# metno/mi-fieldcalc

Hardware: AMD Instinct MI355X
Metric: Mcells/s fused vorticity+divergence, 1440x720x137 grid; % HBM roofline (higher is better)
Workload: dtype f32 in/out, f64 combine; 1 GPU; 1440x720x137 float32 fused relvort+divergence (BASELINE.json configs[2]), one 137-level ensemble member per GPU, inputs ALL_DEFINED and resident in HBM; nx=1440, ny=720, nlev=137, members_per_gpu=1, tuning=default, level_stride_floats=1036800

## Files before the change

include/mifc.h:

```cpp
#ifndef MIFC_H
#define MIFC_H

#include <stddef.h>

#ifdef __cplusplus
extern "C" {
#endif

#define MIFC_ABI_VERSION 1

enum { MIFC_ALL_DEFINED = 0, MIFC_NONE_DEFINED = 1, MIFC_SOME_DEFINED = 2 };
enum { MIFC_MEM_HOST = 0, MIFC_MEM_DEVICE = 1 };

typedef struct mifc_ctx mifc_ctx;

int mifc_abi_version(void);
int mifc_device_count(void);
mifc_ctx* mifc_create(int device);
void mifc_destroy(mifc_ctx* ctx);
const char* mifc_last_error(const mifc_ctx* ctx);
int mifc_set_stream(mifc_ctx* ctx, void* hip_stream);
int mifc_use_own_stream(mifc_ctx* ctx);
int mifc_synchronize(mifc_ctx* ctx);
int mifc_not_built(mifc_ctx* ctx, const char* what);
// ... 156 lines not shown
                             const float* airtemp, const float* rh, const float* sst, const float* p, const float* Pw, const float* aice,
                             const float* depth, float vs, float alpha, float zmin, float zmax, float* icing, int* fdefined, float undef,
                             int memkind);
int mifc_vesselIcingMincog(mifc_ctx* ctx, int nx, int ny, const float* sal, const float* wave, const float* x_wind, const float* y_wind,
                           const float* airtemp, const float* rh, const float* sst, const float* p, const float* Pw, const float* aice,
                           const float* depth, float vs, float alpha, float zmin, float zmax, int alt, float* icing, int* fdefined, float undef,
                           int memkind);
enum { MIFC_ICING_MODSTALL = 1, MIFC_ICING_MINCOG = 2 };
int mifc_vesselIcing_levels(mifc_ctx* ctx, int model, int nlev, int nx, int ny, const float* sal, const float* wave, const float* x_wind,
                            const float* y_wind, const float* airtemp, const float* rh, const float* sst, const float* p, const float* Pw,
                            const float* aice, const float* depth, unsigned int shared_mask, float vs, float alpha, float zmin, float zmax, int alt,
                            float* icing, int* fdefined, float undef, int memkind);

int mifc_vortdiv_levels(mifc_ctx* ctx, int nx, int ny, int nlev, const float* u, const float* v, const float* xmapr, const float* ymapr,
                        float* rvort, float* diverg, int* fdefined, float undef, int memkind);
int mifc_vortdiv_levels_enqueue(mifc_ctx* ctx, int nx, int ny, int nlev, const float* u, const float* v, const float* xmapr, const float* ymapr,
                                float* rvort, float* diverg, const int* fdefined_in, float undef, unsigned long long* n_undefined_dev);

size_t mifc_batch_level_stride(int nx, int ny);
int mifc_vortdiv_levels_strided_enqueue(mifc_ctx* ctx, int nx, int ny, int nlev, const float* u, const float* v, const float* xmapr,
                                        const float* ymapr, float* rvort, float* diverg, size_t in_level_stride, size_t out_level_stride,
                                        const int* fdefined_in, float undef, unsigned long long* n_undefined_dev);

int mifc_vortdiv_ff_levels_enqueue(mifc_ctx* ctx, int nx, int ny, int nlev, const float* u, const float* v, const float* xmapr,
                                   const float* ymapr, float* rvort, float* diverg, float* ff, const int* fdefined_in, float undef,
                                   unsigned long long* n_undefined_dev, unsigned long long* n_undefined_ff_dev);

enum {
  MIFC_OP_RELVORT = 0, MIFC_OP_ABSVORT = 1, MIFC_OP_DIVERGENCE = 2, MIFC_OP_VORTDIV = 3,
  MIFC_OP_GRADIENT_X = 4, MIFC_OP_GRADIENT_Y = 5, MIFC_OP_GRADIENT_ABS = 6, MIFC_OP_GRADIENT_LAPLACE = 7,
  MIFC_OP_GWIND_X = 8, MIFC_OP_GWIND_Y = 9, MIFC_OP_GVORT = 10, MIFC_OP_IGWIND = 11,
  MIFC_OP_JACOBIAN = 13,
  MIFC_OP_ADVECTION = 12, MIFC_OP_TFP = 14, MIFC_OP_QVECTOR = 15, MIFC_OP_SHAPIRO2 = 17
};
int mifc_stencil_levels(mifc_ctx* ctx, int op, int nx, int ny, int nlev, const float* f0, const float* f1, const float* xmapr, const float* ymapr,
                        const float* fcoriolis, float* out0, float* out1, int* fdefined, float undef, int memkind);

int mifc_stencil_levels_enqueue(mifc_ctx* ctx, int op, int nx, int ny, int nlev, const float* f0, const float* f1, const float* xmapr,
                                const float* ymapr, const float* fcoriolis, float* out0, float* out1, const int* fdefined_in, float undef,
                                unsigned long long* n_undefined_dev);
unsigned long long mifc_stencil_count_domain(int op, int nx, int ny);

const char* mifc_last_stencil_form(void);

int mifc_stencil_levels_ex(mifc_ctx* ctx, int op, int nx, int ny, int nlev, const float* f0, const float* f1, const float* f2, const float* xmapr,
                           const float* ymapr, const float* fcoriolis, const float* level_scalars, float scalar, int compute, float* out0,
// ... 61 lines not shown
```

include/mifc_measure.h:

```cpp
#ifndef MIFC_MEASURE_H
#define MIFC_MEASURE_H

#include "mifc.h"

#ifdef __cplusplus
extern "C" {
#endif

int mifc_timing_begin(mifc_ctx* ctx);
float mifc_timing_end_ms(mifc_ctx* ctx);
int mifc_bench_stream2(mifc_ctx* ctx, int variant, int blocks, float* dst0, float* dst1, const float* src0, const float* src1,
                       size_t n_floats);

int mifc_diag_division(mifc_ctx* ctx, const float* a, const float* b, const float* g, float* shared, float* plain, size_t n);

#ifdef __cplusplus
}
#endif

#endif
```

mi-fieldcalc_amd/_capi.py:

```python
import ctypes
import os

_HERE = os.path.dirname(os.path.abspath(__file__))
LIB_PATH = os.environ.get("MIFC_LIB_PATH") or os.path.join(_HERE, "libmifc.so")

c_float_p = ctypes.POINTER(ctypes.c_float)
c_int_p = ctypes.POINTER(ctypes.c_int)
c_u64_p = ctypes.POINTER(ctypes.c_ulonglong)

_T = {
    "ctx": ctypes.c_void_p,
    "i": ctypes.c_int,
    "f": ctypes.c_float,
    "fl": ctypes.c_float,
    "s": ctypes.c_char_p,
    "p": ctypes.c_void_p,
    "pi": ctypes.c_void_p,
    "pu": ctypes.c_void_p,
    "z": ctypes.c_size_t,
    "u64": ctypes.c_ulonglong,
}

SIGNATURES = {
    "mifc_abi_version": ("i", []),
    "mifc_device_count": ("i", []),
    "mifc_create": ("ctx", ["i"]),
    "mifc_destroy": (None, ["ctx"]),
    "mifc_last_error": ("s", ["ctx"]),
    "mifc_set_stream": ("i", ["ctx", "p"]),
    "mifc_use_own_stream": ("i", ["ctx"]),
    "mifc_synchronize": ("i", ["ctx"]),
    "mifc_reload_env": ("i", ["ctx"]),
    "mifc_not_built": ("i", ["ctx", "s"]),
    "mifc_device_alloc": ("p", ["ctx", "z"]),
    "mifc_device_free": ("i", ["ctx", "p"]),
# ... 69 lines not shown
    "mifc_fieldOPERconstant": ("i", ["ctx", "i", "i", "i", "p", "f", "p", "pi", "f", "i"]),
    "mifc_constantOPERfield": ("i", ["ctx", "i", "i", "i", "f", "p", "p", "pi", "f", "i"]),
    "mifc_sumFields": ("i", ["ctx", "i", "i", "p", "i", "p", "pi", "f", "i"]),
    "mifc_meanValue": ("i", ["ctx", "i", "i", "p", "p", "i", "p", "pi", "f", "i"]),
    "mifc_stddevValue": ("i", ["ctx", "i", "i", "p", "p", "i", "p", "pi", "f", "i"]),
    "mifc_extremeValue": ("i", ["ctx", "i", "i", "i", "p", "i", "p", "pi", "f", "i"]),
    "mifc_probability": ("i", ["ctx", "i", "i", "i", "p", "p", "i", "p", "i", "p", "pi", "f", "i"]),
    "mifc_ensembleQuantiles": ("i", ["ctx", "i", "i", "i", "i", "p", "pi", "i", "p", "i", "p", "pi", "f", "i"]),
    "mifc_neighbourProbFunctions": ("i", ["ctx", "i", "i", "p", "p", "i", "i", "p", "pi", "f", "i"]),
    "mifc_neighbourFunctions": ("i", ["ctx", "i", "i", "p", "p", "i", "i", "p", "pi", "f", "i"]),
    "mifc_neighbour_levels": ("i", ["ctx", "i", "i", "i", "i", "i", "p", "p", "i", "p", "pi", "f", "i"]),
    "mifc_vesselIcingModStall": ("i", ["ctx", "i", "i"] + ["p"] * 11 + ["f", "f", "f", "f", "p", "pi", "f", "i"]),
    "mifc_vesselIcingMincog": ("i", ["ctx", "i", "i"] + ["p"] * 11 + ["f", "f", "f", "f", "i", "p", "pi", "f", "i"]),
    "mifc_vesselIcing_levels": ("i", ["ctx", "i", "i", "i", "i"] + ["p"] * 11 + ["i", "f", "f", "f", "f", "i", "p", "pi", "f", "i"]),
    "mifc_vortdiv_levels": ("i", ["ctx", "i", "i", "i", "p", "p", "p", "p", "p", "p", "pi", "f", "i"]),
    "mifc_stencil_levels": ("i", ["ctx", "i", "i", "i", "i", "p", "p", "p", "p", "p", "p", "p", "pi", "f", "i"]),
    "mifc_vortdiv_ff_levels_enqueue": ("i", ["ctx", "i", "i", "i", "p", "p", "p", "p", "p", "p", "p", "pi", "f", "pu", "pu"]),
    "mifc_stencil_levels_enqueue": ("i", ["ctx", "i", "i", "i", "i", "p", "p", "p", "p", "p", "p", "p", "pi", "f", "pu"]),
    "mifc_stencil_count_domain": ("u64", ["i", "i", "i"]),
    "mifc_last_stencil_form": ("s", []),
    "mifc_stencil_levels_ex": ("i", ["ctx", "i", "i", "i", "i", "p", "p", "p", "p", "p", "p", "p", "f", "i", "p", "p", "pi", "f", "i"]),
    "mifc_vortdiv_levels_enqueue": ("i", ["ctx", "i", "i", "i", "p", "p", "p", "p", "p", "p", "pi", "f", "pu"]),
    "mifc_batch_level_stride": ("z", ["i", "i"]),
    "mifc_vortdiv_levels_strided_enqueue": ("i", ["ctx", "i", "i", "i", "p", "p", "p", "p", "p", "p", "z", "z", "pi", "f", "pu"]),
    "mifc_hlevel_derived_levels": (
        "i",
        ["ctx", "i", "i", "i", "p", "p", "p", "p", "p", "p", "p", "p", "p", "p", "pi", "pi", "pi", "pi", "pi", "f", "i"],
    ),
    "mifc_hlevel_derived_levels_enqueue": (
        "i",
        ["ctx", "i", "i", "i", "p", "p", "p", "p", "p", "p", "p", "p", "p", "p", "pi", "pi", "f", "pu"],
    ),
    "mifc_hlevel_derived_batch": (
        "i",
        ["ctx", "i", "i", "i", "p", "p", "p", "p", "p", "p", "p", "p", "p", "s", "i", "p", "s", "i", "p", "s", "i", "p", "pi", "pi", "pi", "pi", "pi",
         "pi", "pi", "f", "i"],
    ),
    "mifc_hlevel_derived_batch_enqueue": (
        "i",
        ["ctx", "i", "i", "i", "p", "p", "p", "p", "p", "p", "p", "p", "p", "s", "i", "p", "s", "i", "p", "s", "i", "p", "pi", "pi", "f", "pu"],
    ),
    "mifc_vortdiv_slab_enqueue": ("i", ["ctx", "i", "i", "i", "i", "p", "p", "p", "p", "p", "p", "i", "f", "pu"]),
    "mifc_vortdiv_slab_rows_enqueue": ("i", ["ctx", "i", "i", "i", "i", "i", "i", "p", "p", "p", "p", "p", "p", "i", "f", "pu", "i"]),
    "mifc_halo_copy_enqueue": ("i", ["ctx", "p", "ctx", "p", "z"]),
    "mifc_graph_begin": ("i", ["ctx", "i"]),
    "mifc_graph_begin_lanes": ("i", ["ctx", "i", "i"]),
    "mifc_graph_lane": ("i", ["ctx", "i"]),
    "mifc_graph_end": ("p", ["ctx"]),
    "mifc_graph_launch": ("i", ["p"]),
    "mifc_graph_destroy": (None, ["p"]),
    "mifc_comm_unique_id": ("i", ["p"]),
    "mifc_comm_init": ("i", ["ctx", "p", "i", "i"]),
    "mifc_comm_adopt": ("i", ["ctx", "p"]),
    "mifc_comm_release": ("i", ["ctx"]),
    "mifc_comm_info": ("i", ["ctx", "pi", "pi"]),
    "mifc_slab_plan_create": ("p", ["ctx", "i", "i", "i", "i", "i", "p", "p", "p", "p", "p", "p", "i", "f", "pu"]),
    "mifc_slab_plan_destroy": (None, ["p"]),
    "mifc_slab_plan_step": ("i", ["p"]),
    "mifc_slab_plan_uses_graph": ("i", ["p"]),
    "mifc_slab_plan_begin": ("i", ["p"]),
    "mifc_slab_plan_finish": ("i", ["p"]),
}


MEASURE_SIGNATURES = {
    "mifc_timing_begin": ("i", ["ctx"]),
    "mifc_timing_end_ms": ("fl", ["ctx"]),
    "mifc_bench_stream2": ("i", ["ctx", "i", "i", "p", "p", "p", "p", "z"]),
    "mifc_diag_division": ("i", ["ctx", "p", "p", "p", "p", "p", "z"]),
}


def load_library(path=LIB_PATH):
    if not os.path.exists(path):
        raise ImportError(
            "%s not found: build the HIP extension first (python -c 'import __graft_entry__ as g; g.build()' "
            "or make -C mi-fieldcalc_amd). There is no CPU fallback." % path
        )
    try:
        import torch
    except ImportError:
        pass
    lib = ctypes.CDLL(path)
    for name, (res, args) in SIGNATURES.items():
        fn = getattr(lib, name)
        fn.restype = _T[res] if res else None
        fn.argtypes = [_T[a] for a in args]
    for name, (res, args) in MEASURE_SIGNATURES.items():
        fn = getattr(lib, name, None)
        if fn is not None:
            fn.restype = _T[res] if res else None
            fn.argtypes = [_T[a] for a in args]
# ... 12 lines not shown
```

mi-fieldcalc_amd/csrc/mifc_capi.hip:

```cpp

#include <cmath>
#include <cstdio>
#include <cstdlib>
#include <cstring>
#include <new>
#include <string>
#include <vector>

#include "mifc_ctx.h"

namespace mifc_host {

void stencil_partials(mifc_ctx* c, mifc::StencilParams& P)
{
  P.partials = nullptr;
  P.partials_cap = 0;
  if (P.every_level_all_defined || c->capturing)
    return;
  const size_t per_level = (size_t)(P.ny_local / 4 + 2) * (size_t)(P.nx / 256 + 1);
  const size_t units = per_level * (size_t)P.nlev;
  if (per_level < 2048 || units > ((size_t)1 << 24))
    return;
  int cap = 0;
  P.partials = partials_for(c, units * 1024, &cap);
// ... 1297 lines not shown
  if (timed) {
    (void)hipEventRecord(c->tev[2 * c->n_timed + 1], c->stream);
    c->n_timed += 1;
  }
  if (e != hipSuccess) {
    fail(c, "mifc_vortdiv_ff_levels_enqueue: launch", e);
    return 0;
  }
  if (!every_all && !scratch_release(c))
    return 0;
  return 1;
}

const char* mifc_last_stencil_form(void)
{
  return mifc::last_form();
}

unsigned long long mifc_stencil_count_domain(int op, int nx, int ny)
{
  return stencil_denominator(op, nx, ny);
}

size_t mifc_batch_level_stride(int nx, int ny)
{
  if (nx <= 0 || ny <= 0)
    return 0;
  return mifc::padded_level_stride((size_t)nx * (size_t)ny);
}

static int stencil_enqueue(mifc_ctx* c, const char* who, mifc::StencilParams& P, const int* fdefined_in, unsigned long long* n_undefined_dev)
{
  if (!ensure_levels(c, (size_t)P.nlev))
    return 0;
  bool every_all = (fdefined_in != nullptr), any_all = false;
  for (int l = 0; l < P.nlev; ++l) {
    const bool a = fdefined_in && fdefined_in[l] == MIFC_ALL_DEFINED;
    every_all = every_all && a;
    any_all = any_all || a;
  }
  P.every_level_all_defined = every_all ? 1 : 0;
  P.all_defined = any_all ? c->d_flags : nullptr;
  P.n_undefined = n_undefined_dev;
  if (!every_all && !n_undefined_dev) {
    c->err = std::string(who) + ": n_undefined_dev is required unless every level is ALL_DEFINED";
    return 0;
// ... 511 lines not shown
  if (src_ctx->device == dst_ctx->device)
    MIFC_HIP(dst_ctx, hipMemcpyAsync(dst_dev, src_dev, n_floats * sizeof(float), hipMemcpyDeviceToDevice, dst_ctx->stream));
  else
    MIFC_HIP(dst_ctx, hipMemcpyPeerAsync(dst_dev, dst_ctx->device, src_dev, src_ctx->device, n_floats * sizeof(float), dst_ctx->stream));
  return 1;
}

#ifdef MIFC_MEASUREMENT_BUILD
int mifc_bench_stream2(mifc_ctx* c, int variant, int blocks, float* dst0, float* dst1, const float* src0, const float* src1, size_t n_floats)
{
  CTX_OR_FAIL(c);
  if (n_floats % 4 != 0)
    return 0;
  MIFC_HIP(c, mifc::launch_stream2(variant, blocks, dst0, dst1, src0, src1, n_floats, c->stream));
  return 1;
}

int mifc_diag_division(mifc_ctx* c, const float* a, const float* b, const float* g, float* shared, float* plain, size_t n)
{
  CTX_OR_FAIL(c);
  MIFC_HIP(c, mifc::launch_division_check(a, b, g, shared, plain, n, c->stream));
  return 1;
}
#endif

}
```

mi-fieldcalc_amd/csrc/mifc_kernels.h:

```cpp
#ifndef MIFC_KERNELS_H
#define MIFC_KERNELS_H

#include <hip/hip_runtime.h>

#include "mifc_env.h"

namespace mifc {

typedef unsigned long long u64;

enum EwiseOp {
  EW_VECTORABS = 0,
  EW_TEMP = 1,
  EW_HUM = 2,
  EW_CVHUM_TD = 3,
  EW_CVHUM_RH = 4,
  EW_MOMENTUM_X = 5,
  EW_MOMENTUM_Y = 6,
  EW_TEMP_SCALAR = 7,
  EW_TEMP_PLAIN = 8,
  EW_HUM_DIRECT = 9
};
enum PressureSource { PS_SCALAR = 0, PS_HYBRID = 1, PS_FIELD = 2 };
enum HumKind { HUM_Q_RH = 0, HUM_RH_Q = 1, HUM_Q_TD = 2, HUM_RH_TD = 3 };
// ... 13 lines not shown
  float p;
  float pidcp;
  float pi;
  float tconv;
  float tdconv;
  float alevel, blevel;
  float unit_scale;
  int nx;
  int cell0;
  float fcormin;
  float undef;
  const float* in0;
  const float* in1;
  const float* in2;
  float* out;
  u64* n_undefined;
  unsigned int* partials;
  int partials_cap;
};

hipError_t launch_ewise(const EwiseParams& prm, hipStream_t stream);

size_t padded_level_stride(size_t n);

struct DerivedParams
{
  int n;
  int nlev;
  const float *u, *v, *t, *h, *ps;
  const float *alevel, *blevel;
  float *ff, *temp, *hum, *td;
  float* dd;
  int temp_compute;
  int hum_code, td_code;
  float hum_tdconv, td_tdconv;
  const unsigned char* wind_all_defined;
  const unsigned char* thermo_all_defined;
  int every_level_all_defined;
  float undef;
  u64 *cnt_ff, *cnt_temp, *cnt_hum, *cnt_td, *cnt_dd;
  int n_inline;
  float a_inline[8], b_inline[8];
  unsigned char wind_inline[8], thermo_inline[8];
};
hipError_t launch_derived_levels(const DerivedParams& prm, hipStream_t stream);

// ... 289 lines not shown
```

mi-fieldcalc_amd/csrc/mifc_vortdiv.hip:

```cpp
#include "mifc_device.h"
#include "mifc_kernels.h"

#include <cstdlib>
#include <cstring>
#include <type_traits>

namespace mifc {

namespace {

struct RowsParams
{
  int nx;
  int nyg;
  int j0;
  int ny_local;
  int lo, hi;
  int R;
  int nbands, nwc, nlev;
  int wpb;
  int uL, uB, uW;
  int n_logical;
  int per_xcd;
  int order;
  int xcd_remap;
  int zigzag;
  int nt_interior;
  int lgroup;
#ifdef MIFC_MEASUREMENT_BUILD
  int exp_nohalo;
  int exp_nostore;
  int exp_noload;
  int exp_store_aux;
#endif
  long idx_lo, idx_hi;
  const float *u, *v, *xm, *ym;
  const float* fc;
  float *rv, *dv;
  float* ff;
  u64* n_undefined_ff;
  long in_stride, out_stride;
  const unsigned char* all_defined;
  float undef;
  u64* n_undefined;
  unsigned int* partials;
};

typedef float v4f __attribute__((ext_vector_type(4)));

__device__ __forceinline__ float dpp_from_lower_lane(float keep_if_none, float x)
{
  return __builtin_bit_cast(float,
// ... 845 lines not shown
            if (bottom)
              store4<NT>(dv + oo + nx, d4);
          }
        }
        if (CHECK && P.n_undefined && !all && __builtin_amdgcn_ballot_w64(bad != 0) != 0) {
          const unsigned int n = wave_sum(bad);
          if (lane == 0)
            atomicAdd(&sbad[(lev - lev0) & 1], n);
        }
      }
    }
  }
chunk_done:;
  if (CHECK) {
    asm volatile("s_waitcnt lgkmcnt(0)\n\ts_barrier" ::: "memory");
    if (P.n_undefined && threadIdx.x == 0 && lev1 > lev0) {
      const unsigned int n = sbad[(lev1 - 1 - lev0) & 1];
      if (n != 0)
        atomicAdd(P.n_undefined + (lev1 - 1), (u64)n);
    }
  }
}

template <bool CHECK, bool NT, int TR, int NL, int PF, bool WANT_V = true, bool WANT_D = true, bool ABSV = false, bool FF = false, bool RAGGED = false,
          bool JAC = false>
__global__ __launch_bounds__(64 * (TR + NL)) void vortdiv_split_kernel(const RowsParams P)
{
  static_assert(WANT_V || WANT_D, "nothing to compute");
  static_assert(!JAC || (WANT_V && !WANT_D && !ABSV && !FF), "the Jacobian is a single-output operator");
  static_assert(!(RAGGED && FF), "the three-output form takes aligned fields only");
  static_assert(!FF || (WANT_V && WANT_D && !ABSV), "the wind speed rides on the fused pair");
  static_assert(!ABSV || (WANT_V && !WANT_D), "absvort is a single-output operator");
  constexpr int NB = PF + 1;
  constexpr int NS = TR + 2;
  constexpr int KMAX = (NS + NL - 1) / NL;
  static_assert(4 * NS <= 64, "the edge scalars of a level are one dword per lane");
  static_assert(NL >= 2, "loader 0 gathers the edge scalars, the last loader hands the undefined counts over");
  __shared__ v4f srow[NB][NS][2][64];
  __shared__ float sedge[NB][64];
  __shared__ unsigned int sbad[2];
  __shared__ unsigned int sbadf[2];
  if (CHECK && threadIdx.x < 2) {
    sbad[threadIdx.x] = 0;
    sbadf[threadIdx.x] = 0;
  }
  const int wave = __builtin_amdgcn_readfirstlane((int)(threadIdx.x >> 6));
  const int lane = threadIdx.x & 63;
  const int bid = blockIdx.x;
  const int seq = P.xcd_remap ? ((bid & 7) * P.per_xcd + (bid >> 3)) : bid;
  if (seq >= P.n_logical)
    return;
  const int ntiles = P.uB * P.uW;
  const int lchunk = seq / ntiles;
  const int tile = seq - lchunk * ntiles;
  const int rblock = tile / P.uW;
  const int wc = tile - rblock * P.uW;
  const int lev0 = lchunk * P.lgroup;
  const int lev1 = (lev0 + P.lgroup < P.nlev) ? lev0 + P.lgroup : P.nlev;
  const int nx = P.nx;
  const int first = P.lo + rblock * TR;
  const int col = wc * 256 + lane * 4;
  const bool act = col < nx;
  const int col_c = act ? col : (RAGGED ? 0 : nx - 4);
  const int nvalid = RAGGED ? ((nx - col) < 4 ? (nx - col) : 4) : 4;
  int east_col = wc * 256 + 256;
  if (east_col > nx)
    east_col = nx;

  if (wave >= TR) {
    const int lw = wave - TR;
    int off[KMAX], slot_of[KMAX];
    int off_end[KMAX];
    bool fix[KMAX];
#pragma unroll
    for (int k = 0; k < KMAX; ++k) {
      int s = lw + NL * k;
      if (s > NS - 1)
        s = NS - 1;
      const int jl_raw = first + s - 1;
      const int jl = jl_raw < P.hi ? jl_raw : P.hi;
      slot_of[k] = s;
      off[k] = jl * nx + col_c;
      fix[k] = RAGGED && ((long)off[k] + 3 > P.idx_hi);
      off_end[k] = fix[k] ? (int)P.idx_hi - 3 : off[k];
    }
    const int ei = (lane < 4 * NS) ? lane : 0;
    const int es = ei >> 2;
    const bool e_is_v = ((ei >> 1) & 1) != 0;
    const int ejl_raw = first + es - 1;
    const int ejl = ejl_raw < P.hi ? ejl_raw : P.hi;
    long e64 = (long)ejl * nx + ((ei & 1) ? east_col : (wc * 256 - 1));
    e64 = e64 < P.idx_lo ? P.idx_lo : (e64 > P.idx_hi ? P.idx_hi : e64);
    const int eoff = (int)e64;
    const float* __restrict__ ebase = e_is_v ? P.v : P.u;

    auto walk = [&](auto edge_tag) __attribute__((always_inline)) {
      constexpr bool EDGE = decltype(edge_tag)::value;
      constexpr int L = 2 * KMAX + (EDGE ? 1 : 0);
      auto issue = [&](int lev, int b) {
        const int l = lev < lev1 ? lev : lev1 - 1;
        const float* __restrict__ u = P.u + (size_t)l * P.in_stride;
        const float* __restrict__ v = P.v + (size_t)l * P.in_stride;
        const bool at_end = RAGGED && l == P.nlev - 1;
#pragma unroll
        for (int k = 0; k < KMAX; ++k) {
          const int o = at_end ? off_end[k] : off[k];
          __builtin_amdgcn_global_load_lds((const void __attribute__((address_space(1)))*)(u + o),
                                           (void __attribute__((address_space(3)))*)&srow[b][slot_of[k]][0][0], 16, 0, 0);
          __builtin_amdgcn_global_load_lds((const void __attribute__((address_space(1)))*)(v + o),
                                           (void __attribute__((address_space(3)))*)&srow[b][slot_of[k]][1][0], 16, 0, 0);
        }
        if (EDGE)
          __builtin_amdgcn_global_load_lds((const void __attribute__((address_space(1)))*)(ebase + (size_t)l * P.in_stride + eoff),
                                           (void __attribute__((address_space(3)))*)&sedge[b][0], 4, 0, 0);
        if constexpr (RAGGED) {
          bool mine = false;
#pragma unroll
          for (int k = 0; k < KMAX; ++k)
            mine = mine | fix[k];
          if (at_end && __builtin_amdgcn_ballot_w64(mine) != 0) {
            asm volatile("s_waitcnt vmcnt(0)" ::: "memory");
#pragma unroll
            for (int k = 0; k < KMAX; ++k) {
              if (fix[k]) {
                v4f qu = {0.f, 0.f, 0.f, 0.f}, qv = qu;
#pragma unroll
                for (int c = 0; c < 4; ++c) {
                  const long i = (long)off[k] + c;
                  if (i <= P.idx_hi) {
                    qu[c] = u[i];
                    qv[c] = v[i];
                  }
                }
                srow[b][slot_of[k]][0][lane] = qu;
                srow[b][slot_of[k]][1][lane] = qv;
              }
            }
          }
        }
      };
#pragma unroll
      for (int k = 0; k < PF; ++k)
        issue(lev0 + k, k);
      int b_next = PF % NB;
      auto hand_over = [&](int lev_done) {
        if (CHECK && !EDGE && lw == NL - 1 && P.n_undefined && lane == 0) {
          const int q = (lev_done - lev0) & 1;
          const unsigned int n = sbad[q];
          if (P.partials) {
            P.partials[(size_t)lev_done * (size_t)ntiles + tile] = n;
            if (n != 0)
              sbad[q] = 0;
          } else if (n != 0) {
            atomicAdd(P.n_undefined + lev_done, (u64)n);
            sbad[q] = 0;
          }
          if constexpr (FF) {
            const unsigned int nf = sbadf[q];
            if (nf != 0) {
              atomicAdd(P.n_undefined_ff + lev_done, (u64)nf);
              sbadf[q] = 0;
            }
          }
        }
      };
      for (int lev = lev0; lev < lev1; ++lev) {
        asm volatile("s_waitcnt vmcnt(%0) lgkmcnt(0)\n\ts_barrier" ::"n"((PF - 1) * L) : "memory");
        issue(lev + PF, b_next);
        b_next = (b_next + 1 == NB) ? 0 : b_next + 1;
        if (lev > lev0)
          hand_over(lev - 1);
      }
      asm volatile("s_waitcnt vmcnt(0)" ::: "memory");
      if (CHECK) {
        asm volatile("s_barrier" ::: "memory");
        if (lev1 > lev0)
          hand_over(lev1 - 1);
      }
    };
    if (lw == 0)
      walk(std::true_type());
    else
      walk(std::false_type());
    return;
  }

  const int slot = wave + 1;
  const int jl_raw = first + wave;
  const bool computes = jl_raw < P.hi;
  const int jl = computes ? jl_raw : P.hi;
  const int j = P.j0 + jl;
  const float undef = P.undef;
  const int base = jl * nx;
  const int o = base + col_c;
  const bool top = (j == 1) && (P.j0 == 0);
  const bool bottom = (j == P.nyg - 2) && (P.j0 + P.ny_local == P.nyg);
  const bool last_in_seg = col + 4 >= east_col;
  const int oo = base + col;
  v4f xm4 = {0.f, 0.f, 0.f, 0.f}, ym4 = xm4, fc4 = xm4;
  if (computes) {
    if constexpr (RAGGED) {
      xm4 = reinterpret_cast<const V4Unaligned*>(P.xm + o)->v;
      ym4 = reinterpret_cast<const V4Unaligned*>(P.ym + o)->v;
      if constexpr (ABSV)
        fc4 = reinterpret_cast<const V4Unaligned*>(P.fc + o)->v;
    } else {
      xm4 = load4(P.xm + o);
      ym4 = load4(P.ym + o);
      if constexpr (ABSV)
        fc4 = load4(P.fc + o);
    }
  }
  const int k_last = nx - 1 - col;
  auto fill_columns = [&](float (&z)[4]) __attribute__((always_inline)) {
    if (col == 0)
      z[0] = z[1];
    if constexpr (RAGGED) {
      const float below = dpp_from_lower_lane(z[3], z[3]);
      if (k_last == 0)
        z[0] = below;
      else if (k_last == 1)
        z[1] = z[0];
      else if (k_last == 2)
// ... 26 lines not shown
          store4<NT>(field + oo + nx, z4);
      }
    }
  };
  float hx4[4] = {0.f, 0.f, 0.f, 0.f}, hy4[4] = {0.f, 0.f, 0.f, 0.f};
  bool halves = false;
  if constexpr (JAC) {
    bool exact = true;
#pragma unroll
    for (int k = 0; k < 4; ++k) {
      hx4[k] = 0.5f * xm4[k];
      hy4[k] = 0.5f * ym4[k];
      exact = exact & (__builtin_fabsf(xm4[k]) >= 0x1p-125f || xm4[k] == 0.f) & (__builtin_fabsf(ym4[k]) >= 0x1p-125f || ym4[k] == 0.f);
    }
    halves = __builtin_amdgcn_ballot_w64(!exact) == 0;
  }
  int buf = 0;
  for (int lev = lev0; lev < lev1; ++lev) {
    bool all = true;
    if (CHECK)
      all = level_flag_then_barrier(P.all_defined, lev);
    else
      asm volatile("s_waitcnt lgkmcnt(0)\n\ts_barrier" ::: "memory");
    if (computes) {
      const v4f uc = srow[buf][slot][0][lane], vc = srow[buf][slot][1][lane];
      const float uWe = sedge[buf][4 * slot + 0], uEe = sedge[buf][4 * slot + 1];
      const float vWe = sedge[buf][4 * slot + 2], vEe = sedge[buf][4 * slot + 3];
      const float uW = dpp_from_lower_lane(uWe, uc.w), vW = dpp_from_lower_lane(vWe, vc.w);
      float uE = dpp_from_upper_lane(uEe, uc.x), vE = dpp_from_upper_lane(vEe, vc.x);
      if (last_in_seg) {
        uE = uEe;
        vE = vEe;
      }
      bool ok[4] = {true, true, true, true};
      unsigned int bad = 0;
      if constexpr (JAC) {
        const v4f un = srow[buf][slot + 1][0][lane], us = srow[buf][slot - 1][0][lane];
        const v4f vn = srow[buf][slot + 1][1][lane], vs = srow[buf][slot - 1][1][lane];
        const float ucx[6] = {uW, uc.x, uc.y, uc.z, uc.w, uE};
        const float vcx[6] = {vW, vc.x, vc.y, vc.z, vc.w, vE};
        bool dux[6] = {true, true, true, true, true, true}, dvx[6] = {true, true, true, true, true, true};
        if (CHECK) {
#pragma unroll
          for (int k = 0; k < 6; ++k) {
            dux[k] = __builtin_islessgreater(ucx[k], undef);
            dvx[k] = __builtin_islessgreater(vcx[k], undef);
// ... 87 lines not shown
            f4.x = f[0];
            f4.y = f[1];
            f4.z = f[2];
            f4.w = f[3];
            store4<NT>(ffp + at, f4);
          }
        };
        speed_row(uc, vc, oo);
        if (top)
          speed_row(srow[buf][slot - 1][0][lane], srow[buf][slot - 1][1][lane], oo - nx);
        if (bottom)
          speed_row(srow[buf][slot + 1][0][lane], srow[buf][slot + 1][1][lane], oo + nx);
        if (CHECK && P.n_undefined_ff && !all && __builtin_amdgcn_ballot_w64(badf != 0) != 0) {
          const unsigned int n = wave_sum(badf);
          if (lane == 0)
            atomicAdd(&sbadf[(lev - lev0) & 1], n);
        }
      }
    }
    buf = (buf + 1 == NB) ? 0 : buf + 1;
  }
  if (CHECK)
    asm volatile("s_waitcnt lgkmcnt(0)\n\ts_barrier" ::: "memory");
}

struct Tuning
{
  int K;
  int R;
  int D;
  int NT;
  int V;
  int ORDER;
  int XCD;
  int WPB;
  int ZZ;
  int NTI;
  int XH;
  int XS;
  int PADROWS;
  int XL;
  int LDSX;
  int STA;
  int LG;
  int RB;
};

int tune_value(const char* s, const char* key, int dflt)
{
  const size_t n = std::strlen(key);
  for (const char* p = s; p && *p;) {
    if (std::strncmp(p, key, n) == 0 && p[n] == '=')
      return std::atoi(p + n + 1);
    p = std::strchr(p, ',');
    if (p)
      ++p;
  }
  return dflt;
}

Tuning current_tuning(int nx)
{
  Tuning t = {0, 8, 1, 1, 2, 1, 1, 8, 1, 0, 0, 0, 0, 0, 0, 0, 0, 8};
  if (env().has_vortdiv_tune) {
    const char* s = env().vortdiv_tune;
    t.K = tune_value(s, "K", t.K);
    t.R = tune_value(s, "R", t.R);
    t.D = tune_value(s, "D", t.D);
    t.NT = tune_value(s, "NT", t.NT);
    t.V = tune_value(s, "V", t.V);
    t.ORDER = tune_value(s, "ORDER", t.ORDER);
    t.XCD = tune_value(s, "XCD", t.XCD);
    t.WPB = tune_value(s, "WPB", t.WPB);
    t.ZZ = tune_value(s, "ZZ", t.ZZ);
    t.NTI = tune_value(s, "NTI", t.NTI);
    t.LDSX = tune_value(s, "LDSX", t.LDSX);
    t.LG = tune_value(s, "LG", t.LG);
    t.RB = tune_value(s, "RB", t.RB);
#ifdef MIFC_MEASUREMENT_BUILD
    t.XH = tune_value(s, "XH", 0);
    t.XS = tune_value(s, "XS", 0);
    t.PADROWS = tune_value(s, "PADROWS", 0);
    t.XL = tune_value(s, "XL", 0);
    t.STA = tune_value(s, "STA", 0);
#endif
  }
  if (t.WPB != 1 && t.WPB != 2 && t.WPB != 4 && t.WPB != 8)
    t.WPB = 4;
  if (t.V != 1 && t.V != 2 && t.V != 3)
    t.V = 2;
  if (nx <= 256)
    t.V = 1;
  if (t.R < 1)
    t.R = 1;
  const int rmax = 32 / t.V;
  if (t.R > rmax)
    t.R = rmax;
  if (t.D < 0)
    t.D = 0;
  if (t.D > 1)
    t.D = 1;
  return t;
}

template <bool CHECK, bool WV, bool WD, bool ABSV, int D, bool NT>
void launch_v(const RowsParams& rp, const Tuning& t, int grid, hipStream_t stream)
{
// ... 34 lines not shown
}

template <bool CHECK>
void launch_outputs(const RowsParams& rp, const Tuning& t, int grid, hipStream_t stream)
{
  if (rp.fc)
    launch_d<CHECK, true, false, true>(rp, t, grid, stream);
  else if (rp.rv && rp.dv)
    launch_d<CHECK, true, true, false>(rp, t, grid, stream);
  else if (rp.rv)
    launch_d<CHECK, true, false, false>(rp, t, grid, stream);
  else
    launch_d<CHECK, false, true, false>(rp, t, grid, stream);
}

constexpr int kLevelWalkMinLevels = 3;
constexpr long kLevelWalkMinUnits = 768;

inline bool aligned16(const void* p)
{
  return (reinterpret_cast<size_t>(p) & 15u) == 0;
}

}

size_t padded_level_stride(size_t n)
{
  const size_t n4 = (n + 3) & ~size_t(3);
  return n4;
}

hipError_t launch_vortdiv_rows(const StencilParams& prm, hipStream_t stream, bool* handled)
{
  *handled = false;
  float* rv = nullptr;
  float* dv = nullptr;
  if (prm.op == ST_VORTDIV) {
    rv = prm.out0;
    dv = prm.out1;
  } else if (prm.op == ST_RELVORT) {
    rv = prm.out0;
  } else if (prm.op == ST_DIVERGENCE) {
    dv = prm.out0;
  } else if (prm.op == ST_ABSVORT) {
    rv = prm.out0;
    if (!prm.fcoriolis)
// ... 67 lines not shown
  }
  const bool has_north_halo = prm.j0 > 0;
  const bool has_south_halo = prm.j0 + rp.ny_local < rp.nyg;
  rp.idx_lo = has_north_halo ? -(long)nx : 0;
  rp.idx_hi = (long)nx * (rp.ny_local + (has_south_halo ? 1 : 0)) - 1;
  rp.R = t.R;
  rp.nbands = (rp.hi - rp.lo + t.R - 1) / t.R;
  rp.nwc = (nx + 256 * t.V - 1) / (256 * t.V);
  rp.nlev = prm.nlev;
  rp.wpb = t.WPB;
  rp.uL = (prm.nlev + t.WPB - 1) / t.WPB;
  rp.uB = rp.nbands;
  rp.uW = rp.nwc;
  const long n_logical = (long)rp.uL * rp.uB * rp.uW;
  if (n_logical > 0x3fffffffL)
    return hipSuccess;
  rp.n_logical = (int)n_logical;
  rp.per_xcd = (rp.n_logical + 7) / 8;
  rp.order = t.ORDER;
  rp.xcd_remap = t.XCD;
  rp.zigzag = t.ZZ;
  rp.nt_interior = t.NTI;
  rp.lgroup = t.LG > 0 ? t.LG : 0;
#ifdef MIFC_MEASUREMENT_BUILD
  rp.exp_nohalo = t.XH;
  rp.exp_nostore = t.XS;
  rp.exp_noload = t.XL;
  rp.exp_store_aux = t.STA;
#endif
  rp.u = prm.f0;
  rp.v = prm.f1;
  rp.xm = prm.xmapr;
  rp.ym = prm.ymapr;
  rp.fc = (prm.op == ST_ABSVORT) ? prm.fcoriolis : nullptr;
  rp.rv = rv;
  rp.dv = dv;
  rp.ff = prm.out_ff;
  rp.n_undefined_ff = prm.n_undefined_ff;
  rp.in_stride = prm.in_level_stride;
  rp.out_stride = prm.out_level_stride;
  rp.all_defined = prm.all_defined;
  rp.undef = prm.undef;
  rp.n_undefined = prm.n_undefined;
  rp.partials = nullptr;
  auto counts_by_partials = [&](long units_per_level, bool level_walking = false) {
    const bool yes = prm.partials && prm.n_undefined && !prm.every_level_all_defined && !prm.out_ff && (level_walking || rp.lgroup == 0) &&
                     units_per_level >= 2048 && units_per_level * prm.nlev <= prm.partials_cap;
// ... 154 lines not shown
      } else if (NWsel == 12 && pf == 2) {
        LEVELWALK(12, 2);
      } else if (NWsel == 12) {
        LEVELWALK(12, 1);
      } else if (pf == 2) {
        LEVELWALK(8, 2);
      } else {
        LEVELWALK(8, 1);
      }
#undef LEVELWALK
      return hipGetLastError();
    }
    *handled = false;
    return hipSuccess;
  }
  if (t.K == 4 && prm.op == ST_JACOBIAN && env().has_vortdiv_tune) {
    *handled = false;
    return hipSuccess;
  }
  if (t.K == 4) {
    const bool single = !(rv && dv) || rp.fc;
    const int tile_rows = (single || ragged || prm.out_ff) ? 12 : ((t.RB == 6 || t.RB == 8 || t.RB == 12 || t.RB == 14) ? t.RB : 10);
    const int nchunks_lg = (t.LG > 0 && t.LG < prm.nlev) ? t.LG : prm.nlev;
    const int nchunks = (prm.nlev + nchunks_lg - 1) / nchunks_lg;
    const long units = (long)nchunks * ((rp.hi - rp.lo + tile_rows - 1) / tile_rows) * ((nx + 255) / 256);
    if (units > 0x3fffffffL || (long)nx * (rp.ny_local + 2) >= 0x7fffffffL) {
      *handled = false;
      return hipSuccess;
    }
    rp.uB = (rp.hi - rp.lo + tile_rows - 1) / tile_rows;
    rp.uW = (nx + 255) / 256;
    rp.lgroup = nchunks_lg;
    rp.n_logical = (int)units;
    rp.per_xcd = (rp.n_logical + 7) / 8;
    grid = rp.per_xcd * 8;
    const bool chk = !prm.every_level_all_defined;
    const bool partials = counts_by_partials((long)rp.uB * rp.uW, true);
    auto finish = [&]() {
      if (partials)
        (void)launch_count_partials_levels(prm.partials, rp.uB * rp.uW, prm.nlev, prm.n_undefined, stream);
      return hipGetLastError();
    };
    const int pf = t.D >= 2 ? 3 : (t.D == 1 ? 2 : 1);
    const int nl = (t.WPB == 2 || t.WPB == 4) ? t.WPB : (tile_rows == 10 ? 4 : 2);
#define SPLIT_AS(TR_, NL_, PF_, ...)                                                                                                       \
  if (chk)                                                                                                                                 \
    hipLaunchKernelGGL((vortdiv_split_kernel<true, true, TR_, NL_, PF_, ##__VA_ARGS__>), dim3(grid), dim3(64 * (TR_ + NL_)), 0, stream, rp); \
  else                                                                                                                                     \
    hipLaunchKernelGGL((vortdiv_split_kernel<false, true, TR_, NL_, PF_, ##__VA_ARGS__>), dim3(grid), dim3(64 * (TR_ + NL_)), 0, stream, rp)
    if (prm.out_ff) {
      SPLIT_AS(12, 2, 2, true, true, false, true);
      return finish();
    }
    if (prm.op == ST_JACOBIAN) {
      if (ragged) {
        SPLIT_AS(12, 2, 2, true, false, false, false, true, true);
      } else {
// ... 123 lines not shown
```

Baseline: 374,200 Mcells/s.

## Add balanced level-chunk planning and drain-tail pipeline for split vortdiv kernel

Adds a cost-based planner that picks how many level chunks to split the 137 levels into so work divides evenly across CUs. It also adds a class-based block decoder that spreads long and short chunks and narrow edge columns evenly across XCDs. The loader loop gets a drain tail that no longer issues dead prefetch loads past the chunk end, plus optional masking of loads from inactive lanes. Most of this sits behind tuning keys (BAL, DL, ML) that default to 0. The default path now skips dead prefetches and uses the new tail waits, and it gains measurement-only timing probes.

```diff
diff --git a/include/mifc.h b/include/mifc.h
--- a/include/mifc.h
+++ b/include/mifc.h
@@ -202,6 +202,8 @@
                                         const float* ymapr, float* rvort, float* diverg, size_t in_level_stride, size_t out_level_stride,
                                         const int* fdefined_in, float undef, unsigned long long* n_undefined_dev);
 
+int mifc_plan_level_chunks(long tiles, int nlev, int cus, int* first_level, int cap);
+
 int mifc_vortdiv_ff_levels_enqueue(mifc_ctx* ctx, int nx, int ny, int nlev, const float* u, const float* v, const float* xmapr,
                                    const float* ymapr, float* rvort, float* diverg, float* ff, const int* fdefined_in, float undef,
                                    unsigned long long* n_undefined_dev, unsigned long long* n_undefined_ff_dev);
diff --git a/include/mifc_measure.h b/include/mifc_measure.h
--- a/include/mifc_measure.h
+++ b/include/mifc_measure.h
@@ -14,6 +14,8 @@
 
 int mifc_diag_division(mifc_ctx* ctx, const float* a, const float* b, const float* g, float* shared, float* plain, size_t n);
 
+void mifc_measure_split_probe(unsigned long long* dev);
+
 #ifdef __cplusplus
 }
 #endif
diff --git a/mi-fieldcalc_amd/_capi.py b/mi-fieldcalc_amd/_capi.py
--- a/mi-fieldcalc_amd/_capi.py
+++ b/mi-fieldcalc_amd/_capi.py
@@ -11,6 +11,7 @@
 _T = {
     "ctx": ctypes.c_void_p,
     "i": ctypes.c_int,
+    "l": ctypes.c_long,
     "f": ctypes.c_float,
     "fl": ctypes.c_float,
     "s": ctypes.c_char_p,
@@ -126,6 +127,7 @@
     "mifc_stencil_levels_ex": ("i", ["ctx", "i", "i", "i", "i", "p", "p", "p", "p", "p", "p", "p", "f", "i", "p", "p", "pi", "f", "i"]),
     "mifc_vortdiv_levels_enqueue": ("i", ["ctx", "i", "i", "i", "p", "p", "p", "p", "p", "p", "pi", "f", "pu"]),
     "mifc_batch_level_stride": ("z", ["i", "i"]),
+    "mifc_plan_level_chunks": ("i", ["l", "i", "i", "pi", "i"]),
     "mifc_vortdiv_levels_strided_enqueue": ("i", ["ctx", "i", "i", "i", "p", "p", "p", "p", "p", "p", "z", "z", "pi", "f", "pu"]),
     "mifc_hlevel_derived_levels": (
         "i",
@@ -172,6 +174,7 @@
     "mifc_timing_end_ms": ("fl", ["ctx"]),
     "mifc_bench_stream2": ("i", ["ctx", "i", "i", "p", "p", "p", "p", "z"]),
     "mifc_diag_division": ("i", ["ctx", "p", "p", "p", "p", "p", "z"]),
+    "mifc_measure_split_probe": (None, ["pu"]),
 }
 
 
diff --git a/mi-fieldcalc_amd/csrc/mifc_capi.hip b/mi-fieldcalc_amd/csrc/mifc_capi.hip
--- a/mi-fieldcalc_amd/csrc/mifc_capi.hip
+++ b/mi-fieldcalc_amd/csrc/mifc_capi.hip
@@ -1343,6 +1343,19 @@
   return stencil_denominator(op, nx, ny);
 }
 
+int mifc_plan_level_chunks(long tiles, int nlev, int cus, int* first_level, int cap)
+{
+  if (tiles < 1 || nlev < 1 || cus < 1)
+    return 0;
+  const int n = mifc::plan_level_chunks(tiles, nlev, cus);
+  if (first_level) {
+    const int q = nlev / n, rem = nlev % n;
+    for (int c = 0; c <= n && c < cap; ++c)
+      first_level[c] = c * q + (c < rem ? c : rem);
+  }
+  return n;
+}
+
 size_t mifc_batch_level_stride(int nx, int ny)
 {
   if (nx <= 0 || ny <= 0)
@@ -1900,6 +1913,11 @@
   MIFC_HIP(c, mifc::launch_division_check(a, b, g, shared, plain, n, c->stream));
   return 1;
 }
+
+void mifc_measure_split_probe(unsigned long long* dev)
+{
+  mifc::set_split_probe(dev);
+}
 #endif
 
 }
diff --git a/mi-fieldcalc_amd/csrc/mifc_kernels.h b/mi-fieldcalc_amd/csrc/mifc_kernels.h
--- a/mi-fieldcalc_amd/csrc/mifc_kernels.h
+++ b/mi-fieldcalc_amd/csrc/mifc_kernels.h
@@ -59,6 +59,10 @@
 hipError_t launch_ewise(const EwiseParams& prm, hipStream_t stream);
 
 size_t padded_level_stride(size_t n);
+int plan_level_chunks(long tiles, int nlev, int cus);
+#ifdef MIFC_MEASUREMENT_BUILD
+void set_split_probe(unsigned long long* dev);
+#endif
 
 struct DerivedParams
 {
diff --git a/mi-fieldcalc_amd/csrc/mifc_vortdiv.hip b/mi-fieldcalc_amd/csrc/mifc_vortdiv.hip
--- a/mi-fieldcalc_amd/csrc/mifc_vortdiv.hip
+++ b/mi-fieldcalc_amd/csrc/mifc_vortdiv.hip
@@ -27,7 +27,13 @@
   int zigzag;
   int nt_interior;
   int lgroup;
+  int nchunks;
+  int cls_n[4];
+  int dead_loads;
+  int mask_lanes;
 #ifdef MIFC_MEASUREMENT_BUILD
+  int exp_nodead;
+  unsigned long long* probe;
   int exp_nohalo;
   int exp_nostore;
   int exp_noload;
@@ -919,6 +925,89 @@
   }
 }
 
+struct SplitUnit
+{
+  int lchunk, rblock, wc, lev0, lev1;
+  bool valid;
+};
+__device__ __forceinline__ SplitUnit decode_split_unit(const RowsParams& P, int bid)
+{
+  SplitUnit U;
+  U.valid = false;
+  U.lchunk = U.rblock = U.wc = U.lev0 = U.lev1 = 0;
+  if (P.nchunks > 0) {
+    const int x = bid & 7;
+    int k = bid >> 3, cls = -1;
+#pragma unroll
+    for (int c = 0; c < 4; ++c) {
+      const long n = P.cls_n[c];
+      const int s0 = (int)((x * n) >> 3), s1 = (int)(((x + 1) * n) >> 3);
+      if (cls < 0) {
+        if (k < s1 - s0) {
+          cls = c;
+          k += s0;
+        } else {
+          k -= s1 - s0;
+        }
+      }
+    }
+    if (cls < 0)
+      return U;
+    const bool narrow = cls >= 2, shorter = (cls & 1) != 0;
+    const int has_narrow = (P.cls_n[2] + P.cls_n[3]) > 0 ? 1 : 0;
+    const int wcount = narrow ? 1 : P.uW - has_narrow;
+    const int per_chunk = P.uB * wcount;
+    const int cc = k / per_chunk;
+    const int t = k - cc * per_chunk;
+    U.rblock = t / wcount;
+    U.wc = (narrow ? P.uW - 1 : 0) + (t - U.rblock * wcount);
+    const int q = P.nlev / P.nchunks, rem = P.nlev - q * P.nchunks;
+    U.lchunk = cc + (shorter ? rem : 0);
+    U.lev0 = U.lchunk * q + (U.lchunk < rem ? U.lchunk : rem);
+    U.lev1 = U.lev0 + q + (U.lchunk < rem ? 1 : 0);
+    U.valid = true;
+    return U;
+  }
+  const int seq = P.xcd_remap ? ((bid & 7) * P.per_xcd + (bid >> 3)) : bid;
+  if (seq >= P.n_logical)
+    return U;
+  const int ntiles = P.uB * P.uW;
+  U.lchunk = seq / ntiles;
+  const int tile = seq - U.lchunk * ntiles;
+  U.rblock = tile / P.uW;
+  U.wc = tile - U.rblock * P.uW;
+  U.lev0 = U.lchunk * P.lgroup;
+  U.lev1 = (U.lev0 + P.lgroup < P.nlev) ? U.lev0 + P.lgroup : P.nlev;
+  U.valid = true;
+  return U;
+}
+
+#ifdef MIFC_MEASUREMENT_BUILD
+unsigned long long* g_split_probe = nullptr;
+inline unsigned long long* split_probe_buffer()
+{
+  return g_split_probe;
+}
+constexpr int kSplitProbeWords = 16;
+__device__ __forceinline__ unsigned long long probe_now()
+{
+  return __builtin_amdgcn_s_memtime();
+}
+#define SPLIT_PROBE(word, value)            \
+  do {                                      \
+    if (P.probe && pw >= 0 && lane == 0)    \
+      sprobe[pw][word] = (value);           \
+  } while (0)
+#define SPLIT_PROBE_FLUSH()                                                                  \
+  do {                                                                                       \
+    if (P.probe && pw >= 0 && lane < kSplitProbeWords)                                       \
+      P.probe[((size_t)bid * 3 + pw) * kSplitProbeWords + lane] = sprobe[pw][lane];          \
+  } while (0)
+#else
+#define SPLIT_PROBE(word, value) ((void)0)
+#define SPLIT_PROBE_FLUSH() ((void)0)
+#endif
+
 template <bool CHECK, bool NT, int TR, int NL, int PF, bool WANT_V = true, bool WANT_D = true, bool ABSV = false, bool FF = false, bool RAGGED = false,
           bool JAC = false>
 __global__ __launch_bounds__(64 * (TR + NL)) void vortdiv_split_kernel(const RowsParams P)
@@ -941,23 +1030,30 @@
     sbad[threadIdx.x] = 0;
     sbadf[threadIdx.x] = 0;
   }
+#ifdef MIFC_MEASUREMENT_BUILD
+  const unsigned long long t_start = probe_now();
+#endif
   const int wave = __builtin_amdgcn_readfirstlane((int)(threadIdx.x >> 6));
   const int lane = threadIdx.x & 63;
   const int bid = blockIdx.x;
-  const int seq = P.xcd_remap ? ((bid & 7) * P.per_xcd + (bid >> 3)) : bid;
-  if (seq >= P.n_logical)
+  const SplitUnit U = decode_split_unit(P, bid);
+  if (!U.valid)
     return;
+#ifdef MIFC_MEASUREMENT_BUILD
+  __shared__ unsigned long long sprobe[3][kSplitProbeWords];
+  const int pw = wave == TR ? 0 : (wave == TR + NL - 1 ? 1 : (wave == 0 ? 2 : -1));
+  if (P.probe && pw >= 0 && lane < kSplitProbeWords)
+    sprobe[pw][lane] = 0;
+#endif
   const int ntiles = P.uB * P.uW;
-  const int lchunk = seq / ntiles;
-  const int tile = seq - lchunk * ntiles;
-  const int rblock = tile / P.uW;
-  const int wc = tile - rblock * P.uW;
-  const int lev0 = lchunk * P.lgroup;
-  const int lev1 = (lev0 + P.lgroup < P.nlev) ? lev0 + P.lgroup : P.nlev;
+  const int rblock = U.rblock, wc = U.wc;
+  const int tile = rblock * P.uW + wc;
+  const int lev0 = U.lev0, lev1 = U.lev1;
   const int nx = P.nx;
   const int first = P.lo + rblock * TR;
   const int col = wc * 256 + lane * 4;
   const bool act = col < nx;
+  const bool ld_act = act || !P.mask_lanes;
   const int col_c = act ? col : (RAGGED ? 0 : nx - 4);
   const int nvalid = RAGGED ? ((nx - col) < 4 ? (nx - col) : 4) : 4;
   int east_col = wc * 256 + 256;
@@ -999,13 +1095,15 @@
         const float* __restrict__ u = P.u + (size_t)l * P.in_stride;
         const float* __restrict__ v = P.v + (size_t)l * P.in_stride;
         const bool at_end = RAGGED && l == P.nlev - 1;
-#pragma unroll
-        for (int k = 0; k < KMAX; ++k) {
-          const int o = at_end ? off_end[k] : off[k];
-          __builtin_amdgcn_global_load_lds((const void __attribute__((address_space(1)))*)(u + o),
-                                           (void __attribute__((address_space(3)))*)&srow[b][slot_of[k]][0][0], 16, 0, 0);
-          __builtin_amdgcn_global_load_lds((const void __attribute__((address_space(1)))*)(v + o),
-                                           (void __attribute__((address_space(3)))*)&srow[b][slot_of[k]][1][0], 16, 0, 0);
+        if (ld_act) {
+#pragma unroll
+          for (int k = 0; k < KMAX; ++k) {
+            const int o = at_end ? off_end[k] : off[k];
+            __builtin_amdgcn_global_load_lds((const void __attribute__((address_space(1)))*)(u + o),
+                                             (void __attribute__((address_space(3)))*)&srow[b][slot_of[k]][0][0], 16, 0, 0);
+            __builtin_amdgcn_global_load_lds((const void __attribute__((address_space(1)))*)(v + o),
+                                             (void __attribute__((address_space(3)))*)&srow[b][slot_of[k]][1][0], 16, 0, 0);
+          }
         }
         if (EDGE)
           __builtin_amdgcn_global_load_lds((const void __attribute__((address_space(1)))*)(ebase + (size_t)l * P.in_stride + eoff),
@@ -1036,9 +1134,11 @@
           }
         }
       };
+      const bool dead = P.dead_loads != 0;
 #pragma unroll
       for (int k = 0; k < PF; ++k)
-        issue(lev0 + k, k);
+        if (dead || lev0 + k < lev1)
+          issue(lev0 + k, k);
       int b_next = PF % NB;
       auto hand_over = [&](int lev_done) {
         if (CHECK && !EDGE && lw == NL - 1 && P.n_undefined && lane == 0) {
@@ -1061,12 +1161,39 @@
           }
         }
       };
-      for (int lev = lev0; lev < lev1; ++lev) {
+      int lev = lev0;
+      for (; lev + PF < lev1; ++lev) {
         asm volatile("s_waitcnt vmcnt(%0) lgkmcnt(0)\n\ts_barrier" ::"n"((PF - 1) * L) : "memory");
+        SPLIT_PROBE(lev == lev0 ? 1 : 2, probe_now());
+        if (lev - lev0 < 8)
+          SPLIT_PROBE(8 + lev - lev0, probe_now());
         issue(lev + PF, b_next);
         b_next = (b_next + 1 == NB) ? 0 : b_next + 1;
         if (lev > lev0)
           hand_over(lev - 1);
+      }
+#pragma unroll
+      for (int r = PF - 1; r >= 0; --r) {
+        if (lev1 - lev0 > r) {
+          bool keep_wait = dead;
+#ifdef MIFC_MEASUREMENT_BUILD
+          keep_wait = keep_wait || P.exp_nodead != 0;
+#endif
+          if (keep_wait)
+            asm volatile("s_waitcnt vmcnt(%0) lgkmcnt(0)\n\ts_barrier" ::"n"((PF - 1) * L) : "memory");
+          else
+            asm volatile("s_waitcnt vmcnt(%0) lgkmcnt(0)\n\ts_barrier" ::"n"(r * L) : "memory");
+          SPLIT_PROBE(lev == lev0 ? 1 : 2, probe_now());
+          if (lev - lev0 < 8)
+            SPLIT_PROBE(8 + lev - lev0, probe_now());
+          if (dead) {
+            issue(lev + PF, b_next);
+            b_next = (b_next + 1 == NB) ? 0 : b_next + 1;
+          }
+          if (lev > lev0)
+            hand_over(lev - 1);
+          ++lev;
+        }
       }
       asm volatile("s_waitcnt vmcnt(0)" ::: "memory");
       if (CHECK) {
@@ -1074,7 +1201,21 @@
         if (lev1 > lev0)
           hand_over(lev1 - 1);
       }
+      SPLIT_PROBE(3, probe_now());
+      SPLIT_PROBE_FLUSH();
     };
+#ifdef MIFC_MEASUREMENT_BUILD
+    {
+      SPLIT_PROBE(0, t_start);
+      unsigned hw, xcc;
+      asm volatile("s_getreg_b32 %0, hwreg(HW_REG_HW_ID)" : "=s"(hw));
+      asm volatile("s_getreg_b32 %0, hwreg(HW_REG_XCC_ID)" : "=s"(xcc));
+      SPLIT_PROBE(4, (unsigned long long)hw);
+      SPLIT_PROBE(5, (unsigned long long)xcc);
+      SPLIT_PROBE(6, (unsigned long long)(lev1 - lev0));
+      SPLIT_PROBE(7, (unsigned long long)(((unsigned)U.lchunk << 20) | ((unsigned)rblock << 8) | (unsigned)wc));
+    }
+#endif
     if (lw == 0)
       walk(std::true_type());
     else
@@ -1095,7 +1236,7 @@
   const bool last_in_seg = col + 4 >= east_col;
   const int oo = base + col;
   v4f xm4 = {0.f, 0.f, 0.f, 0.f}, ym4 = xm4, fc4 = xm4;
-  if (computes) {
+  if (computes && ld_act) {
     if constexpr (RAGGED) {
       xm4 = reinterpret_cast<const V4Unaligned*>(P.xm + o)->v;
       ym4 = reinterpret_cast<const V4Unaligned*>(P.ym + o)->v;
@@ -1168,6 +1309,13 @@
       all = level_flag_then_barrier(P.all_defined, lev);
     else
       asm volatile("s_waitcnt lgkmcnt(0)\n\ts_barrier" ::: "memory");
+#ifdef MIFC_MEASUREMENT_BUILD
+    if (wave == 0) {
+      SPLIT_PROBE(lev == lev0 ? 1 : 2, probe_now());
+      if (lev - lev0 < 8)
+        SPLIT_PROBE(8 + lev - lev0, probe_now());
+    }
+#endif
     if (computes) {
       const v4f uc = srow[buf][slot][0][lane], vc = srow[buf][slot][1][lane];
       const float uWe = sedge[buf][4 * slot + 0], uEe = sedge[buf][4 * slot + 1];
@@ -1301,6 +1449,14 @@
   }
   if (CHECK)
     asm volatile("s_waitcnt lgkmcnt(0)\n\ts_barrier" ::: "memory");
+#ifdef MIFC_MEASUREMENT_BUILD
+  if (wave == 0) {
+    SPLIT_PROBE(0, t_start);
+    SPLIT_PROBE(3, probe_now());
+    SPLIT_PROBE(6, (unsigned long long)(lev1 - lev0));
+    SPLIT_PROBE_FLUSH();
+  }
+#endif
 }
 
 struct Tuning
@@ -1323,6 +1479,11 @@
   int STA;
   int LG;
   int RB;
+  int DL;
+  int BAL;
+  int ML;
+  int NC;
+  int XDL;
 };
 
 int tune_value(const char* s, const char* key, int dflt)
@@ -1340,7 +1501,7 @@
 
 Tuning current_tuning(int nx)
 {
-  Tuning t = {0, 8, 1, 1, 2, 1, 1, 8, 1, 0, 0, 0, 0, 0, 0, 0, 0, 8};
+  Tuning t = {0, 8, 1, 1, 2, 1, 1, 8, 1, 0, 0, 0, 0, 0, 0, 0, 0, 8, 0, 0, 0, 0, 0};
   if (env().has_vortdiv_tune) {
     const char* s = env().vortdiv_tune;
     t.K = tune_value(s, "K", t.K);
@@ -1356,12 +1517,17 @@
     t.LDSX = tune_value(s, "LDSX", t.LDSX);
     t.LG = tune_value(s, "LG", t.LG);
     t.RB = tune_value(s, "RB", t.RB);
+    t.DL = tune_value(s, "DL", t.DL);
 #ifdef MIFC_MEASUREMENT_BUILD
     t.XH = tune_value(s, "XH", 0);
     t.XS = tune_value(s, "XS", 0);
     t.PADROWS = tune_value(s, "PADROWS", 0);
     t.XL = tune_value(s, "XL", 0);
     t.STA = tune_value(s, "STA", 0);
+    t.BAL = tune_value(s, "BAL", 0);
+    t.ML = tune_value(s, "ML", 0);
+    t.NC = tune_value(s, "NC", 0);
+    t.XDL = tune_value(s, "XDL", 0);
 #endif
   }
   if (t.WPB != 1 && t.WPB != 2 && t.WPB != 4 && t.WPB != 8)
@@ -1442,6 +1608,58 @@
   return (reinterpret_cast<size_t>(p) & 15u) == 0;
 }
 
+}
+
+constexpr int kChunkStartLevels = 1;
+int plan_level_chunks(long tiles, int nlev, int cus)
+{
+  if (nlev < 1)
+    return 1;
+  const int target = nlev >= 48 ? 6 : 8;
+  const int n0 = (nlev + target - 1) / target;
+  if (tiles < 1 || cus < 1)
+    return n0;
+  int best = n0;
+  long best_cost = -1;
+  for (int n = 1; n <= nlev; ++n) {
+    const int q = nlev / n, rem = nlev % n;
+    const int longest = q + (rem ? 1 : 0);
+    if ((longest > target + 1 || q < target - 1) && n != n0)
+      continue;
+    const long rounds = (tiles * n + cus - 1) / cus;
+    const long long_rounds = rem ? (tiles * rem + cus - 1) / cus : 0;
+    const long cost = long_rounds * (q + 1 + kChunkStartLevels) + (rounds - long_rounds) * (q + kChunkStartLevels);
+    const int d = n > n0 ? n - n0 : n0 - n, dbest = best > n0 ? best - n0 : n0 - best;
+    if (best_cost < 0 || cost < best_cost || (cost == best_cost && d < dbest)) {
+      best = n;
+      best_cost = cost;
+    }
+  }
+  return best;
+}
+
+#ifdef MIFC_MEASUREMENT_BUILD
+void set_split_probe(unsigned long long* dev)
+{
+  g_split_probe = dev;
+}
+#endif
+
+namespace {
+int device_cus()
+{
+  static int cached[64];
+  int dev = 0;
+  if (hipGetDevice(&dev) != hipSuccess || dev < 0 || dev >= 64)
+    return 256;
+  int n = __atomic_load_n(&cached[dev], __ATOMIC_RELAXED);
+  if (n <= 0) {
+    if (hipDeviceGetAttribute(&n, hipDeviceAttributeMultiprocessorCount, dev) != hipSuccess || n <= 0)
+      n = 256;
+    __atomic_store_n(&cached[dev], n, __ATOMIC_RELAXED);
+  }
+  return n;
+}
 }
 
 size_t padded_level_stride(size_t n)
@@ -1555,7 +1773,13 @@
   rp.zigzag = t.ZZ;
   rp.nt_interior = t.NTI;
   rp.lgroup = t.LG > 0 ? t.LG : 0;
+  rp.nchunks = 0;
+  rp.cls_n[0] = rp.cls_n[1] = rp.cls_n[2] = rp.cls_n[3] = 0;
+  rp.dead_loads = t.DL != 0;
+  rp.mask_lanes = t.ML != 0;
 #ifdef MIFC_MEASUREMENT_BUILD
+  rp.exp_nodead = t.XDL;
+  rp.probe = split_probe_buffer();
   rp.exp_nohalo = t.XH;
   rp.exp_nostore = t.XS;
   rp.exp_noload = t.XL;
@@ -1756,8 +1980,15 @@
     const bool single = !(rv && dv) || rp.fc;
     const int tile_rows = (single || ragged || prm.out_ff) ? 12 : ((t.RB == 6 || t.RB == 8 || t.RB == 12 || t.RB == 14) ? t.RB : 10);
     const int nchunks_lg = (t.LG > 0 && t.LG < prm.nlev) ? t.LG : prm.nlev;
-    const int nchunks = (prm.nlev + nchunks_lg - 1) / nchunks_lg;
-    const long units = (long)nchunks * ((rp.hi - rp.lo + tile_rows - 1) / tile_rows) * ((nx + 255) / 256);
+    const long tiles_k4 = (long)((rp.hi - rp.lo + tile_rows - 1) / tile_rows) * ((nx + 255) / 256);
+    int nchunks = (prm.nlev + nchunks_lg - 1) / nchunks_lg;
+    if (t.BAL)
+      nchunks = plan_level_chunks(tiles_k4, prm.nlev, device_cus());
+#ifdef MIFC_MEASUREMENT_BUILD
+    if (t.BAL && t.NC > 0 && t.NC <= prm.nlev)
+      nchunks = t.NC;
+#endif
+    const long units = (long)nchunks * tiles_k4;
     if (units > 0x3fffffffL || (long)nx * (rp.ny_local + 2) >= 0x7fffffffL) {
       *handled = false;
       return hipSuccess;
@@ -1767,6 +1998,23 @@
     rp.lgroup = nchunks_lg;
     rp.n_logical = (int)units;
     rp.per_xcd = (rp.n_logical + 7) / 8;
+    if (t.BAL) {
+      const int rem = prm.nlev % nchunks;
+      const long longer = rem ? rem : nchunks, shorter = nchunks - longer;
+      const long narrow = (nx % 256 != 0 && rp.uW > 1) ? 1 : 0;
+      rp.nchunks = nchunks;
+      rp.cls_n[0] = (int)(rp.uB * (rp.uW - narrow) * longer);
+      rp.cls_n[1] = (int)(rp.uB * (rp.uW - narrow) * shorter);
+      rp.cls_n[2] = (int)(rp.uB * narrow * longer);
+      rp.cls_n[3] = (int)(rp.uB * narrow * shorter);
+      rp.per_xcd = 0;
+      for (int x = 0; x < 8; ++x) {
+        int mine = 0;
+        for (int c = 0; c < 4; ++c)
+          mine += (int)((((long)x + 1) * rp.cls_n[c]) >> 3) - (int)(((long)x * rp.cls_n[c]) >> 3);
+        rp.per_xcd = mine > rp.per_xcd ? mine : rp.per_xcd;
+      }
+    }
     grid = rp.per_xcd * 8;
     const bool chk = !prm.every_level_all_defined;
     const bool partials = counts_by_partials((long)rp.uB * rp.uW, true);
```

New measurement: 374,000 Mcells/s, median of 2. Within noise of the previous version (-0.1%).
